# rainorangelemon/gnn-motion-planning

Measured on AMD Instinct MI355X. Metric: RGG graphs/sec (GNN explorer forward), 1000-node k=8, higher is better.
Workload: dtype f32; 1 GPU; BASELINE configs[1]: maze2, batch of 256 problems per GPU, 1000-node k1=8 RGGs (mean E=11265, O=116), loop=5, use_obstacles, real weights_maze checkpoint, fp32, sparse per-edge scores; graphs_per_gpu=256, graphs_total=256, parallelism=problem-sharded x1 (256 problems per GPU)

## Files before the change

gnn-motion-planning_amd/csrc/api.cpp:

```cpp
#include <hip/hip_runtime.h>
#include <cmath>
#include <cstdio>
#include <cstdlib>
#include <cstring>
#include <string>
#include <vector>

#include "../../include/gnnmp.h"
#include "kernels.hpp"
#include "layout.hpp"

using namespace gnnmp;

namespace {

thread_local std::string g_hip_error;

int hip_fail(hipError_t e) {
    g_hip_error = hipGetErrorString(e);
    return GNNMP_ERR_HIP;
}

#define HIP_TRY(expr)                              \
    do {                                           \
// ... 215 lines not shown
    struct Rec { int stage; hipEvent_t a, b; };
    std::vector<Rec> recs;
    std::vector<hipEvent_t> pool;
    hipEvent_t get() {
        if (!pool.empty()) { hipEvent_t e = pool.back(); pool.pop_back(); return e; }
        hipEvent_t e = nullptr;
        (void)hipEventCreate(&e);
        return e;
    }
};

struct gnnmp_explorer {
    gnnmp_explorer_dims dims;
    int device;
    float* w_dev;
    ExplorerOffsets off;
    EncBlob enc_e, enc_n;
    ObsBlob obs;
    StageProf* prof;
    int n_cu;
    int resident;
    int resident_both;
    int node_f64;
    float* w_raw_dev;
    std::vector<Entry> man;
    std::vector<int64_t> man_off;
    int64_t n_raw;
};

namespace {
struct StageScope {
    StageProf* p; hipStream_t st; hipEvent_t b = nullptr;
    StageScope(StageProf* p_, int stage, hipStream_t s) : p(p_ && p_->on ? p_ : nullptr), st(s) {
        if (!p) return;
        hipEvent_t a = p->get();
        b = p->get();
        (void)hipEventRecord(a, st);
        p->recs.push_back({stage, a, b});
    }
    ~StageScope() { if (p) (void)hipEventRecord(b, st); }
};
}

extern "C" int gnnmp_explorer_manifest(const gnnmp_explorer_dims* dims, int index, char* name, size_t name_cap,
                                       int64_t* numel) {
    if (!dims) return GNNMP_ERR_NULL;
// ... 235 lines not shown
    if (dims->embed_size == 32) {
        if (P == 2) pack_explorer<32, 2>(B, *dims, h, packed);
        else if (P == 1) pack_explorer<32, 1>(B, *dims, h, packed);
        else pack_explorer<32, 0>(B, *dims, h, packed);
    } else {
        if (P == 2) pack_explorer<64, 2>(B, *dims, h, packed);
        else if (P == 1) pack_explorer<64, 1>(B, *dims, h, packed);
        else pack_explorer<64, 0>(B, *dims, h, packed);
    }
    int prev_dev = -1;
    (void)hipGetDevice(&prev_dev);
    hipError_t e = hipSetDevice(device);
    if (e == hipSuccess) {
        int ncu = 0;
        e = hipDeviceGetAttribute(&ncu, hipDeviceAttributeMultiprocessorCount, device);
        h->n_cu = (ncu > 0 ? ncu : 256) & ~7;
        if (h->n_cu < 8) h->n_cu = 8;
        const char* env = std::getenv("GNNMP_RESIDENT");
        h->resident = !(env && env[0] == '0');
        const char* env2 = std::getenv("GNNMP_PRE_BOTH");
        h->resident_both = !(env2 && env2[0] == '0');
        const char* env3 = std::getenv("GNNMP_NODE_F64");
        h->node_f64 = !(env3 && env3[0] == '0');
    }
    if (e == hipSuccess) e = hipMalloc((void**)&h->w_dev, packed.size() * sizeof(float));
    if (e == hipSuccess) e = hipMemcpy(h->w_dev, packed.data(), packed.size() * sizeof(float), hipMemcpyHostToDevice);
    if (e == hipSuccess) e = hipMalloc((void**)&h->w_raw_dev, (size_t)tot * sizeof(float));
    if (e == hipSuccess) e = hipMemcpy(h->w_raw_dev, weights_host, (size_t)tot * sizeof(float), hipMemcpyHostToDevice);
    if (prev_dev >= 0 && prev_dev != device) (void)hipSetDevice(prev_dev);
    if (e != hipSuccess) {
        if (h->w_dev) (void)hipFree(h->w_dev);
        if (h->w_raw_dev) (void)hipFree(h->w_raw_dev);
        delete h->prof;
        delete h;
        return hip_fail(e);
    }
    *out = h;
    return GNNMP_OK;
}

extern "C" int gnnmp_explorer_destroy(gnnmp_explorer* h) {
    if (!h) return GNNMP_ERR_NULL;
    if (h->w_dev) (void)hipFree(h->w_dev);
    if (h->w_raw_dev) (void)hipFree(h->w_raw_dev);
    if (h->prof) {
        for (auto& r : h->prof->recs) { (void)hipEventDestroy(r.a); (void)hipEventDestroy(r.b); }
// ... 253 lines not shown
    const int* obs_ptr = implicit ? at<int>(ws, c.in_ptrs) + 4 : b->obs_ptr;
    {
    StageScope sc(prof, GNNMP_STAGE_PREP, st);
    q = prep_params(c, b, C, ws, implicit, use_obstacles ? 32 * c.ot_max : 0x7fffffff,
                    status_out ? reinterpret_cast<int*>(status_out) : at<int>(ws, c.gstat));
    HIP_TRY(launch_prep(q, c.Npad, c.Epad, at<int>(ws, c.prep_hist), st));
    if (dense) HIP_TRY(launch_zero_dense(dense, q.dense_ptr + c.G, st));
    if (pre_only) HIP_TRY(t_sort_csr(c.Npad, q.csr, q.row_beg, q.deg, st));
    }

    const bool use_obs = use_obstacles != 0;
    bool use_m0 = false;
    if (use_obs) {
        ObsParams op;
        op.obstacles = b->obstacles; op.obs_ptr = obs_ptr; op.S = h->dims.obs_size;
        op.w[0] = W + h->off.obs_n; op.w[1] = W + h->off.obs_e;
        op.blob = h->obs;
        op.kv[0] = at<float>(ws, c.kv_n); op.kv[1] = at<float>(ws, c.kv_e);
        op.kv_stride = c.kv_stride; op.ot_max = c.ot_max;
        NodeF64Params nq;
        nq.v = b->v; nq.C = C; nq.node_ptr = node_ptr; nq.node_ptr_pad = q.node_ptr_pad; nq.ntile_graph = q.ntile_graph;
        nq.w = W + h->off.f64; nq.blob = F64Blob::make(D, C);
        nq.m0 = at<float>(ws, c.M0);
        nq.groups = c.Npad / 64 > 2 * h->n_cu ? 4 : 1;
        {
            static const char* ord = std::getenv("GNNMP_F64_FIRST");
            nq.f64_first = ord ? (ord[0] != '0') : (nq.groups > 1 && D == 32);
        }
        nq.n_wg = (P != GNNMP_BF16 && h->node_f64) ? c.Npad / (64 * nq.groups) : 0;
        use_m0 = nq.n_wg > 0;
        StageScope sc(prof, GNNMP_STAGE_OBS, st);
        HIP_TRY(launch_obs(D, P, op, nq, c.G, st));
    }

    PreParams pp[2];
    PrePlan plan[2];
    size_t res_lds[2] = {0, 0};
    const size_t res_bytes = ((size_t)3 * (att_staged(D, P) + 6 * vec_floats(D)) + (size_t)3 * c.kv_stride) * sizeof(float) + 64 + 128;
    const bool resident_ok = ((D == 32 && P == 0) || P == 1) && use_obs && res_bytes <= 163840 && h->resident;
    for (int edge = 0; edge < 2; ++edge) {
        PreParams& p = pp[edge];
        p.v = b->v; p.goal = b->goal; p.C = C;
        p.node_ptr = node_ptr; p.node_ptr_pad = q.node_ptr_pad;
        p.tile_graph = edge ? q.etile_graph : q.ntile_graph;
        p.csr = q.csr;
        p.rec32 = at<int>(ws, c.rec32);
        p.obs_ptr = obs_ptr; p.goal_node = q.goal_node;
        p.enc = W + (edge ? h->off.enc_e : h->off.enc_n);
        p.encb = edge ? h->enc_e : h->enc_n;
        p.att = W + (edge ? h->off.att_e : h->off.att_n);
        p.out = W + (edge ? h->off.out_e : h->off.out_n);
        p.out_size = edge ? out_e_size(D, P) : out_n_size(D, P);
// ... 76 lines not shown
    }
    return GNNMP_OK;
}
}

extern "C" int gnnmp_explorer_debug_tap(const gnnmp_explorer* h, const gnnmp_batch* b, int which, float* dst, void* ws,
                                        size_t ws_bytes, void* hip_stream) {
    if (!h || !b || !dst || !ws) return GNNMP_ERR_NULL;
    Carve c;
    if (!carve(h, b, c)) return GNNMP_ERR_ARG;
    if (ws_bytes < c.total) return GNNMP_ERR_WORKSPACE;
    hipStream_t st = static_cast<hipStream_t>(hip_stream);
    const int D = h->dims.embed_size;
    size_t src;
    switch (which) {
        case 0: src = c.XI; break;
        case 1: src = c.H; break;
        case 2:
            if (h->dims.mlp_dtype == GNNMP_BF16) return GNNMP_ERR_DIMS;
            src = c.X; break;
        case 3:
            HIP_TRY(launch_goal_tap(c.G, at<int>(ws, c.goal_node), at<int>(ws, c.node_ptr_pad), dst, st));
            return GNNMP_OK;
        default: return GNNMP_ERR_ARG;
    }
    HIP_TRY(launch_unpad_rows(c.G, b->total_nodes, D, b->node_ptr ? b->node_ptr : at<int>(ws, c.in_ptrs), at<int>(ws, c.node_ptr_pad),
                              at<float>(ws, src), dst, st));
    return GNNMP_OK;
}

namespace {

std::vector<Entry> smoother_manifest(const gnnmp_smoother_dims& d) {
    const int C = d.config_size, D = d.embed_size;
    std::vector<Entry> m;
    auto lin = [&](const std::string& n, int out, int in) {
        m.push_back({n + ".weight", out, in});
        m.push_back({n + ".bias", out, 0});
    };
    lin("node_code.0", D, C + 3);
    m.push_back({"node_code.1.weight", D, 0});
    m.push_back({"node_code.1.bias", D, 0});
    m.push_back({"node_code.1.running_mean", D, 0});
    m.push_back({"node_code.1.running_var", D, 0});
    lin("node_code.3", D, D);
    lin("process.lin_0.0", D, 3 * D);
// ... 1610 lines not shown
TrainGeom to_train_geom(const gnnmp_train_geom* g) {
    TrainGeom q;
    q.G = g->n_graphs; q.C = g->config_size; q.Npad = g->n_pad; q.Epad = g->e_pad;
    q.v = g->v; q.goal = g->goal; q.node_ptr = g->node_ptr; q.node_ptr_pad = g->node_ptr_pad; q.ntile_graph = g->ntile_graph;
    q.goal_node = g->goal_node; q.row_beg = g->row_beg; q.deg = g->deg; q.csr = reinterpret_cast<const int4*>(g->csr);
    q.out_beg = g->out_beg; q.out_cnt = g->out_cnt; q.out_cur = g->out_cur; q.out_slot = g->out_slot;
    return q;
}

struct GeomCarve { Carve c; size_t obeg, ocnt, ocur, oslot, total; };
bool geom_carve(const gnnmp_batch* b, int C, GeomCarve& g) {
    (void)C;
    if (!carve(32, GNNMP_F32, b, g.c)) return false;
    size_t o = g.c.total;
    auto take = [&](size_t bytes) { const size_t r = o; o += (bytes + 255) & ~(size_t)255; return r; };
    g.obeg = take(sizeof(int) * (size_t)g.c.Npad); g.ocnt = take(sizeof(int) * (size_t)g.c.Npad);
    g.ocur = take(sizeof(int) * (size_t)g.c.Npad); g.oslot = take(sizeof(int) * (size_t)g.c.Epad);
    g.total = o;
    return true;
}

}

extern "C" int gnnmp_train_geom_workspace_bytes(const gnnmp_batch* shape, int32_t config_size, size_t* bytes) {
    if (!shape || !bytes) return GNNMP_ERR_NULL;
    if (config_size < 1) return GNNMP_ERR_ARG;
    GeomCarve g;
    if (!geom_carve(shape, config_size, g)) return GNNMP_ERR_ARG;
    *bytes = g.total;
    return GNNMP_OK;
}

extern "C" int gnnmp_train_geom_build(const gnnmp_batch* b, int32_t config_size, void* ws, size_t ws_bytes,
                                      gnnmp_train_geom* out, void* hip_stream) {
    if (!b || !ws || !out) return GNNMP_ERR_NULL;
    if (config_size < 1) return GNNMP_ERR_ARG;
    GeomCarve g;
    if (!geom_carve(b, config_size, g)) return GNNMP_ERR_ARG;
    if (!b->v || !b->goal || !b->node_ptr || !b->edge_ptr || (b->total_edges > 0 && !b->edge_index)) return GNNMP_ERR_NULL;
    if (ws_bytes < g.total || (reinterpret_cast<uintptr_t>(ws) & 255)) return GNNMP_ERR_WORKSPACE;
    hipStream_t st = static_cast<hipStream_t>(hip_stream);
    const Carve& c = g.c;
    const PrepParams q = prep_params(c, b, config_size, ws, false, 0x7fffffff, at<int>(ws, c.gstat));
    HIP_TRY(launch_prep(q, c.Npad, c.Epad, at<int>(ws, c.prep_hist), st));
    HIP_TRY(t_sort_csr(c.Npad, q.csr, q.row_beg, q.deg, st));
    out->n_graphs = c.G; out->config_size = config_size; out->n_pad = c.Npad; out->e_pad = c.Epad;
// ... 137 lines not shown
```

gnn-motion-planning_amd/csrc/explorer_kernels.hip:

```cpp
#include <hip/hip_runtime.h>
#include <cstdio>
#include <cstdlib>
#include <map>
#include <mutex>
#include <utility>
#include <math.h>
#include "chain.hpp"
#include "layout.hpp"
#include "kernels.hpp"

namespace gnnmp {

#define kETile (P == 1 ? 512 : 1024)

__device__ __forceinline__ int round_up(int x, int m) { return (x + m - 1) / m * m; }

__device__ __forceinline__ int find_graph(const int* __restrict__ ptr, int G, int x) {
    int lo = 0, hi = G;
    while (hi - lo > 1) {
        const int mid = (lo + hi) >> 1;
        if (ptr[mid] <= x) lo = mid; else hi = mid;
    }
    return lo;
}
// ... 15 lines not shown
    __syncthreads();
    if (lane == 63) wsum[wave] = x;
    __syncthreads();
    int before = 0, all = 0;
#pragma unroll
    for (int w = 0; w < 16; ++w) {
        const int t = wsum[w];
        before += w < wave ? t : 0;
        all += t;
    }
    total = all;
    return x + before;
}

__device__ __forceinline__ int prep_np(const PrepParams& q, int i) { return q.single_out ? (i > 0 ? q.single_n : 0) : q.node_ptr[i]; }
__device__ __forceinline__ int prep_ep(const PrepParams& q, int i) { return q.single_out ? (i > 0 ? q.single_e : 0) : q.edge_ptr[i]; }

__device__ __forceinline__ int prep_id(int x, int Ng, int& bad) {
    const bool b = (unsigned)x >= (unsigned)Ng;
    bad |= b ? 1 : 0;
    return b ? 0 : x;
}

__device__ __forceinline__ void prep_graph_body(const PrepParams& q, int g, int part, int parts, int n0, int Np, int e0, int e1,
                                                int* prep_lds) {
    __shared__ int carry;
    __shared__ int below_w[16];
    const int tid = threadIdx.x;
    const int c0 = prep_ep(q, g), Eg = prep_ep(q, g + 1) - c0;
    const int span = ((Np + parts - 1) / parts + 31) & ~31;
    const int lo = min(part * span, Np), hi = min(lo + span, Np), Nown = hi - lo;
    const bool in_lds = Nown <= kPrepCap;
    int* cnt = in_lds ? prep_lds : q.deg + n0 + lo;
    int* rb = in_lds ? prep_lds + kPrepCap : q.row_beg + n0 + lo;
    int* scan = prep_lds + 2 * kPrepCap;
    const long long* srcs = q.edge_index + c0;
    const long long* dsts = q.edge_index + (size_t)q.E + c0;
    for (int i = tid; i < Nown; i += 1024) cnt[i] = 0;
    __syncthreads();
    int below = 0;
    constexpr int U = 16;
    const bool in_regs = Eg <= U * 1024;
    const int Ng = prep_np(q, g + 1) - prep_np(q, g);
    int bad_id = 0;
    int sv_r[U], tv_r[U], rk_r[U];
    if (in_regs) {
#pragma unroll
        for (int u = 0; u < U; ++u) {
            const int cc = tid + u * 1024;
            const bool ok = cc < Eg;
            tv_r[u] = ok ? prep_id((int)dsts[cc], Ng, bad_id) : -1;
            sv_r[u] = ok ? prep_id((int)srcs[cc], Ng, bad_id) : 0;
        }
#pragma unroll
        for (int u = 0; u < U; ++u) {
            const int t = tv_r[u];
            below += (t >= 0 && t < lo) ? 1 : 0;
            const bool mine = t >= lo && t < hi;
// ... 3 lines not shown
    } else {
        for (int c = tid; c < Eg; c += U * 1024) {
            int d[U];
#pragma unroll
            for (int u = 0; u < U; ++u) d[u] = (c + u * 1024 < Eg) ? prep_id((int)dsts[c + u * 1024], Ng, bad_id) : 0x7fffffff;
#pragma unroll
            for (int u = 0; u < U; ++u) {
                if (d[u] < lo) ++below;
                else if (d[u] < hi) q.cursor[c0 + c + u * 1024] = atomicAdd(&cnt[d[u] - lo], 1);
            }
        }
    }
#pragma unroll
    for (int off = 32; off > 0; off >>= 1) below += __shfl_down(below, off);
    if ((tid & 63) == 0) below_w[tid >> 6] = below;
    __syncthreads();
    if (tid == 0) {
        int sum = e0;
#pragma unroll
        for (int w = 0; w < 16; ++w) sum += below_w[w];
        carry = sum;
    }
    __syncthreads();
    int carry_run = carry;
    for (int base = 0; base < Nown; base += 1024) {
        const int i = base + tid;
        const int d = (i < Nown) ? cnt[i] : 0;
        int chunk_total;
        const int incl = block_scan_1024(d, scan, chunk_total);
        if (i < Nown) {
            const int r = carry_run + incl - d;
            rb[i] = r;
            if (in_lds) { q.row_beg[n0 + lo + i] = r; q.deg[n0 + lo + i] = d; }
        }
        carry_run += chunk_total;
    }
    __syncthreads();
    if (in_regs) {
#pragma unroll
        for (int u = 0; u < U; ++u)
            if (tv_r[u] >= 0)
                q.csr[rb[tv_r[u] - lo] + rk_r[u]] = make_int4(n0 + sv_r[u], n0 + tv_r[u], c0 + tid + u * 1024, 0);
    } else {
        for (int c = tid; c < Eg; c += U * 1024) {
            int sv[U], tv[U], rk[U];
#pragma unroll
            for (int u = 0; u < U; ++u) {
                const int cc = c + u * 1024;
                tv[u] = cc < Eg ? prep_id((int)dsts[cc], Ng, bad_id) : -1;
            }
#pragma unroll
            for (int u = 0; u < U; ++u) {
                const int cc = c + u * 1024;
                const bool mine = tv[u] >= lo && tv[u] < hi;
                sv[u] = mine ? prep_id((int)srcs[cc], Ng, bad_id) : 0;
                rk[u] = mine ? q.cursor[c0 + cc] : 0;
                if (!mine) tv[u] = -1;
            }
#pragma unroll
            for (int u = 0; u < U; ++u)
                if (tv[u] >= 0)
                    q.csr[rb[tv[u] - lo] + rk[u]] = make_int4(n0 + sv[u], n0 + tv[u], c0 + c + u * 1024, 0);
        }
    }
    if (part == 0)
// ... 95 lines not shown
        an += round_up(ng, kPad);
        ae += round_up(prep_ep(q, t + 1) - prep_ep(q, t), kPad);
        ad += (long long)ng * ng;
    }
#pragma unroll
    for (int off = 32; off > 0; off >>= 1) { an += __shfl_down(an, off); ae += __shfl_down(ae, off); ad += __shfl_down(ad, off); }
    if ((tid & 63) == 0) { red[0][tid >> 6] = an; red[1][tid >> 6] = ae; red[2][tid >> 6] = ad; }
    __syncthreads();
    an = 0; ae = 0; ad = 0;
#pragma unroll
    for (int w = 0; w < 16; ++w) { an += red[0][w]; ae += red[1][w]; ad += red[2][w]; }
    const int ng_own = prep_np(q, g + 1) - prep_np(q, g);
    n0 = (int)an; e0 = (int)ae;
    n1 = n0 + round_up(ng_own, kPad); e1 = e0 + round_up(prep_ep(q, g + 1) - prep_ep(q, g), kPad);
    if (tid == 0 && part == 0) {
        if (g == 0) { q.node_ptr_pad[0] = 0; q.edge_ptr_pad[0] = 0; q.dense_ptr[0] = 0; }
        q.node_ptr_pad[g + 1] = n1; q.edge_ptr_pad[g + 1] = e1; q.dense_ptr[g + 1] = ad + (long long)ng_own * ng_own;
        const int og = q.obs_ptr ? q.obs_ptr[g + 1] - q.obs_ptr[g] : q.single_o;
        q.gstat[kGstatStride * g] = og > q.obs_cap ? 1 : 0;
        for (int pp = parts; pp < kGstatStride - 1; ++pp) q.gstat[kGstatStride * g + 1 + pp] = 0;
    }
}

__device__ __forceinline__ void prep_trailing(const PrepParams& q, int n_end, int e_end, int Npad, int Epad) {
    const int tid = threadIdx.x;
    for (int i = n_end + tid; i < Npad; i += 1024) { q.deg[i] = 0; q.row_beg[i] = e_end; }
    for (int t = n_end / 32 + tid; t < Npad / 32; t += 1024) q.ntile_graph[t] = -1;
    for (int t = e_end / 32 + tid; t < Epad / 32; t += 1024) { q.etile_graph[t] = -1; q.tile_meta[t] = -1; }
    for (int sl = e_end + tid; sl < Epad; sl += 1024) q.csr[sl] = make_int4(-1, -1, -1, -1);
}

__global__ __launch_bounds__(1024) void prep_small_kernel(PrepParams q, int Npad, int Epad, int parts) {
    extern __shared__ int prep_lds[];
    const int g = blockIdx.x / parts, part = blockIdx.x - g * parts;
    int n0, n1, e0, e1;
    prep_prefix<false>(q, g, part, parts, n0, n1, e0, e1);
    prep_graph_body(q, g, part, parts, n0, n1 - n0, e0, e1, prep_lds);
    if (part == 0) goal_body(q.C, q.v, q.goal, prep_np(q, g), prep_np(q, g + 1) - prep_np(q, g), g, n0, q.goal_node);
    if (g == q.G - 1 && part == parts - 1) prep_trailing(q, n1, e1, Npad, Epad);
}

__global__ __launch_bounds__(1024) void prep_hist_kernel(PrepParams q, int Npad, int Epad, int parts, int* __restrict__ H) {
    extern __shared__ int prep_lds[];
    const int idx = blockIdx.x >> 3, g = (idx / parts) * 8 + (blockIdx.x & 7), part = idx % parts, tid = threadIdx.x;
    if (g >= q.G) return;
    int n0, n1, e0, e1;
    prep_prefix<true>(q, g, part, parts, n0, n1, e0, e1);
    const int Np = n1 - n0;
    const int c0 = q.edge_ptr[g], Eg = q.edge_ptr[g + 1] - c0;
    const int cs = (int)((long long)Eg * part / parts), ce = (int)((long long)Eg * (part + 1) / parts);
    int* hslice = H + (size_t)n0 * parts + (size_t)part * Np;
    const bool in_lds = Np <= kPrepCap;
    int* cnt = in_lds ? prep_lds : hslice;
    const long long* dsts = q.edge_index + (size_t)q.E + c0;
    for (int i = tid; i < Np; i += 1024) cnt[i] = 0;
    __syncthreads();
    constexpr int U = 16;
    const int Ng = q.node_ptr[g + 1] - q.node_ptr[g];
    int bad_id = 0;
    for (int c = cs + tid; c < ce; c += U * 1024) {
        int d[U];
#pragma unroll
// ... 296 lines not shown
                y[ob] = __builtin_amdgcn_mfma_f64_16x16x4f64((double)A[((ob * NB + ib) * 4 + st) * 64 + lane], x[ib][st], y[ob], 0, 0, 0);
            if constexpr (NB > 2) __builtin_amdgcn_sched_barrier(0);
        }
}

template <int NB>
__device__ __forceinline__ void vec64(const float* b, f64x4 (&y)[NB], int g) {
#pragma unroll
    for (int ob = 0; ob < NB; ++ob)
#pragma unroll
        for (int r = 0; r < 4; ++r) y[ob][r] = (double)b[16 * ob + 4 * r + g];
}

template <int D, int P>
__device__ __forceinline__ void node_f64_body(const ObsParams& p, const NodeF64Params& q, const int vblock) {
    constexpr int NB = D / 16, NT = D / 32, OC = f64_obs_chunk(D);
    extern __shared__ __attribute__((aligned(16))) float lds[];
    const F64Blob L = q.blob;
    float* wl = lds;
    float* kd = lds + ((L.size + 3) & ~3);
    float* vd = kd + OC * D;
    const int wave = threadIdx.x >> 6, lane = threadIdx.x & 63, j16 = lane & 15, g = lane >> 4;
    const int row00 = vblock * 64 * q.groups;
    const int gr = q.ntile_graph[row00 >> 5];
    if (gr < 0) return;
    stage(wl, q.w, L.size);
    const int o0 = p.obs_ptr[gr], O = min(p.obs_ptr[gr + 1] - o0, p.ot_max * 32);
    const int OT = (O + 31) / 32;
    const int C = q.C;
    const int nbase_pad = q.node_ptr_pad[gr], nbase = q.node_ptr[gr], ng = q.node_ptr[gr + 1] - nbase;
    const bool single_chunk = O <= OC;
    const double isd = 1.0 / sqrt((double)D);
    for (int grp = 0; grp < q.groups; ++grp) {
    const int row0 = row00 + grp * 64;
    if (row0 - nbase_pad >= ng) {
        for (int i = threadIdx.x; i < (q.groups - grp) * 64 * D; i += 256) q.m0[(size_t)row0 * D + i] = 0.f;
        break;
    }
    const int row = row0 + wave * 16 + j16, local = row - nbase_pad;
    const float* vr = q.v + (size_t)(nbase + (local < ng ? local : 0)) * C;

    f64x4 x[NB], acc[NB];
    float xf[NB][4];
    float mxs = 0.f, l0s = 0.f;
    double den = 0.0;
    for (int oc0 = 0; oc0 == 0 || oc0 < O; oc0 += OC) {
        if (oc0 > 0 || (grp > 0 && !single_chunk)) __syncthreads();
        if (grp == 0 || !single_chunk)
        {
            const ObsBlob Lo = p.blob;
            const int h = lane >> 5, j = lane & 31, S = p.S;
            for (int ot = (oc0 >> 5) + wave; ot < min(OT, (oc0 + OC) >> 5); ot += 4) {
                const float* W = p.w[0];
                asm volatile("" : "+s"(W));
                const int o = ot * 32 + j;
                const bool valid = o < O;
                const float* orow = p.obstacles + (size_t)(o0 + (valid ? o : 0)) * S;
                f32x16 code[NT], K[NT], V[NT];
                mlp2_in<NT, P>(W + Lo.as0, Lo.ks, W + Lo.b0, W + Lo.a0, W + Lo.c0,
                               [&](int k) { const bool ok = k < S; const float xx = orow[ok ? k : 0]; return ok ? xx : 0.f; }, code, lane);
#pragma unroll
                for (int t = 0; t < NT; ++t) { K[t] = splat16(0.f); V[t] = splat16(0.f); }
                linear_acc_p<P, NT, NT>(W + Lo.blk0 + Lo.wk, code, K, lane);
                linear_acc_p<P, NT, NT>(W + Lo.blk0 + Lo.wv, code, V, lane);
                const int oo = o - oc0;
                float* kb = kd + (oo >> 4) * NB * 256 + (oo & 15) + 64 * h;
                float* vb = vd + (oo >> 4) * NB * 256 + (oo & 3) * 64 + 16 * ((oo & 15) >> 2) + 4 * h;
#pragma unroll
                for (int t = 0; t < NT; ++t)
#pragma unroll
                    for (int r = 0; r < 16; ++r) {
                        const int f0 = 32 * t + phi(r, 0);
                        kb[(f0 >> 4) * 256 + ((f0 & 15) >> 2) * 64 + 16 * (f0 & 3)] = valid ? K[t][r] : 0.f;
                        vb[(f0 >> 4) * 256 + (f0 & 15)] = valid ? V[t][r] : 0.f;
                    }
            }
        }
        if (grp == 0 || !single_chunk) __syncthreads();
        if (oc0 == 0) {
            f64x4 hdn[NB];
            vec64<NB>(wl + L.b1, hdn, g);
            for (int st = 0; st < L.ks; ++st) {
                const int k = 4 * st + g;
                const double xin = k < C ? (double)vr[k] : 0.0;
#pragma unroll
                for (int ob = 0; ob < NB; ++ob)
                    hdn[ob] = __builtin_amdgcn_mfma_f64_16x16x4f64((double)wl[L.w1 + (ob * L.ks + st) * 64 + lane], xin, hdn[ob], 0, 0, 0);
            }
#pragma unroll
            for (int ob = 0; ob < NB; ++ob)
#pragma unroll
                for (int r = 0; r < 4; ++r) hdn[ob][r] = fmax(hdn[ob][r], 0.0);
            vec64<NB>(wl + L.b2, x, g);
            lin64<NB>(wl + L.w2, hdn, x, lane);
#pragma unroll
            for (int ob = 0; ob < NB; ++ob)
#pragma unroll
                for (int r = 0; r < 4; ++r) xf[ob][r] = (float)x[ob][r];
            f32x4 tq[NB], mv[NB];
#pragma unroll
            for (int ob = 0; ob < NB; ++ob) { tq[ob] = f32x4{0.f, 0.f, 0.f, 0.f}; mv[ob] = f32x4{0.f, 0.f, 0.f, 0.f}; }
// ... 1784 lines not shown
template <class K>
static hipError_t set_lds(K kernel, size_t bytes) {
    return hipFuncSetAttribute(reinterpret_cast<const void*>(kernel), hipFuncAttributeMaxDynamicSharedMemorySize,
                               (int)bytes);
}

int prep_parts(int G, int E) {
    static const int parts_env = getenv("GNNMP_PREP_PARTS") ? atoi(getenv("GNNMP_PREP_PARTS")) : 0;
    const long long g = G > 0 ? G : 1;
    long long parts = (long long)E / (g * kPrepEdgesPerPart);
    if (parts > 256 / g) parts = 256 / g;
    if (parts > 1) {
        long long fine = (long long)E / (g * (kPrepEdgesPerPart / 2));
        if (fine > 512 / g) fine = 512 / g;
        if (fine > 8) fine = 8;
        if (fine > parts) parts = fine;
    }
    if (parts_env > 0) parts = parts_env;
    if (parts < 1) parts = 1;
    if (parts > kPrepMaxParts) parts = kPrepMaxParts;
    return (int)parts;
}

hipError_t launch_prep(const PrepParams& q, int Npad, int Epad, int* hist, hipStream_t st) {
    const size_t glds = (size_t)(2 * kPrepCap + 1024) * sizeof(int);
    const int parts = prep_parts(q.G, q.E);
    if (parts == 1) {
        const hipError_t attr = set_lds(prep_small_kernel, glds);
        if (attr != hipSuccess) return attr;
        static const int slices_env = getenv("GNNMP_PREP_SLICES") ? atoi(getenv("GNNMP_PREP_SLICES")) : 0;
        int slices = q.G > 0 ? 512 / q.G : 1;
        const int by_nodes = q.G > 0 ? (Npad / q.G) / 128 : 1;
        if (slices > by_nodes) slices = by_nodes;
        if (slices > 8) slices = 8;
        if (slices_env > 0) slices = slices_env;
        if (slices < 1) slices = 1;
        if (slices > kGstatStride - 1) slices = kGstatStride - 1;
        hipLaunchKernelGGL(prep_small_kernel, dim3(q.G * slices), dim3(1024), glds, st, q, Npad, Epad, slices);
        LAUNCH_CHECK();
        return hipSuccess;
    }
    hipError_t attr = set_lds(prep_hist_kernel, glds);
    if (attr != hipSuccess) return attr;
    attr = set_lds(prep_scatter_kernel, glds);
    if (attr != hipSuccess) return attr;
    const unsigned grid = (unsigned)(((q.G + 7) / 8) * 8 * parts);
    hipLaunchKernelGGL(prep_hist_kernel, dim3(grid), dim3(1024), glds, st, q, Npad, Epad, parts, hist);
    LAUNCH_CHECK();
    hipLaunchKernelGGL(prep_scatter_kernel, dim3(grid), dim3(1024), glds, st, q, parts, hist, hist + (size_t)parts * Npad);
    LAUNCH_CHECK();
    return hipSuccess;
}


template <int D, int P>
static hipError_t launch_obs_t(const ObsParams& p, const NodeF64Params& q, int G, hipStream_t st) {
    const int f64_blocks = P == 1 ? 0 : q.n_wg;
    size_t lds = f64_blocks ? (size_t)(((q.blob.size + 3) & ~3) + 2 * f64_obs_chunk(D) * D) * sizeof(float) : 0;
    const size_t obs_lds = (D == 32 && P != 2) ? (size_t)((p.blob.size + 3) & ~3) * sizeof(float) : 0;
    if (obs_lds > lds) lds = obs_lds;
    if (lds) {
        const hipError_t e = set_lds(obs_kernel<D, P>, lds);
        if (e != hipSuccess) return e;
    }
    hipLaunchKernelGGL((obs_kernel<D, P>), dim3(f64_blocks + 2 * G), dim3(256), lds, st, p, q, f64_blocks);
    LAUNCH_CHECK();
    return hipSuccess;
}
#define GNNMP_DISPATCH_DP(D_, P_, CALL)                                                     \
    do {                                                                                     \
        if ((D_) == 32 && (P_) == 0) { constexpr int DD = 32, PP = 0; return CALL; }         \
        if ((D_) == 32 && (P_) == 1) { constexpr int DD = 32, PP = 1; return CALL; }         \
        if ((D_) == 32 && (P_) == 2) { constexpr int DD = 32, PP = 2; return CALL; }         \
        if ((D_) == 64 && (P_) == 0) { constexpr int DD = 64, PP = 0; return CALL; }         \
        if ((D_) == 64 && (P_) == 1) { constexpr int DD = 64, PP = 1; return CALL; }         \
        if ((D_) == 64 && (P_) == 2) { constexpr int DD = 64, PP = 2; return CALL; }         \
        return hipErrorInvalidValue;                                                         \
    } while (0)

hipError_t launch_obs(int D, int P, const ObsParams& p, const NodeF64Params& q, int G, hipStream_t st) {
    GNNMP_DISPATCH_DP(D, P, (launch_obs_t<DD, PP>(p, q, G, st)));
}

// ... 43 lines not shown
    return hipErrorInvalidValue;
}
hipError_t launch_pre_resident(int D, int P, bool edge, const PreParams& p, size_t lds_bytes, int n_cu, hipStream_t st) {
    if (D == 32 && P == 0) return edge ? launch_pre_resident_t<32, 0, true, 12>(p, lds_bytes, n_cu, st) : launch_pre_resident_t<32, 0, false, 12>(p, lds_bytes, n_cu, st);
    if (D == 32 && P == 1) return edge ? launch_pre_resident_t<32, 1, true, 12>(p, lds_bytes, n_cu, st) : launch_pre_resident_t<32, 1, false, 12>(p, lds_bytes, n_cu, st);
    if (D == 64 && P == 1) return edge ? launch_pre_resident_t<64, 1, true, 12>(p, lds_bytes, n_cu, st) : launch_pre_resident_t<64, 1, false, 8>(p, lds_bytes, n_cu, st);
    return hipErrorInvalidValue;
}

struct Residency { int per_cu, cus; };
static Residency resident_workgroups(const void* kernel, size_t lds_bytes) {
    static std::mutex mu;
    static std::map<std::pair<const void*, size_t>, Residency> cache;
    std::lock_guard<std::mutex> lock(mu);
    auto it = cache.find({kernel, lds_bytes});
    if (it != cache.end()) return it->second;
    Residency r{0, 256};
    int dev = 0;
    hipDeviceProp_t prop;
    if (hipGetDevice(&dev) == hipSuccess && hipGetDeviceProperties(&prop, dev) == hipSuccess) r.cus = prop.multiProcessorCount;
    if (hipOccupancyMaxActiveBlocksPerMultiprocessor(&r.per_cu, kernel, 256, lds_bytes) != hipSuccess || r.per_cu < 1) r.per_cu = 4;
    if (getenv("GNNMP_DEBUG_GRID")) fprintf(stderr, "[gnnmp] resident workgroups per CU: %d (lds %zu)\n", r.per_cu, lds_bytes);
    return cache[{kernel, lds_bytes}] = r;
}

template <class K>
static int grid_for(K kernel, size_t lds_bytes, int n_tiles, int max_per_cu) {
    int groups = ((n_tiles + 3) / 4 + 7) & ~7;
    if (groups < 8) groups = 8;
    const Residency r = resident_workgroups(reinterpret_cast<const void*>(kernel), lds_bytes);
    int per_cu = r.per_cu < max_per_cu ? r.per_cu : max_per_cu;
    static const int forced = getenv("GNNMP_WGS_PER_CU") ? atoi(getenv("GNNMP_WGS_PER_CU")) : 0;
    if (forced > 0) per_cu = forced;
    const int cap = (r.cus * per_cu) & ~7;
    return groups < cap ? groups : (cap < 8 ? 8 : cap);
}

#ifdef GNNMP_MP_TRACE
static long long* g_mp_trace = nullptr;
static size_t g_mp_trace_n = 0;
extern "C" long long gnnmp_debug_mp_trace(long long* dst, long long cap) {
    if (!g_mp_trace) return 0;
    const size_t n = g_mp_trace_n < (size_t)cap ? g_mp_trace_n : (size_t)cap;
    (void)hipDeviceSynchronize();
    (void)hipMemcpy(dst, g_mp_trace, n * sizeof(long long), hipMemcpyDeviceToHost);
    return (long long)n;
// ... 147 lines not shown
```

gnn-motion-planning_amd/csrc/kernels.hpp:

```cpp
#pragma once
#include <hip/hip_runtime.h>
#include "layout.hpp"

namespace gnnmp {

struct PrepParams {
    int G, E, C;
    const long long* edge_index;
    const int *node_ptr, *edge_ptr;
    const float *v, *goal;
    int *node_ptr_pad, *edge_ptr_pad;
    long long* dense_ptr;
    int *deg, *cursor, *row_beg;
    int *ntile_graph, *etile_graph;
    int4* csr;
    int* goal_node;
    int* tile_meta;
    int2* blk_span;
    int* single_out;
    int single_n, single_e, single_o;
    int n_etiles;
    const int* obs_ptr;
    int obs_cap;
    int* gstat;
};
constexpr int kGstatStride = 17;

struct ObsParams {
    const float* obstacles;
    const int* obs_ptr;
    int S;
    const float* w[2];
    ObsBlob blob;
    float* kv[2];
    int kv_stride;
    int ot_max;
};

struct NodeF64Params {
    const float* v;
    int C;
    const int *node_ptr, *node_ptr_pad, *ntile_graph;
    const float* w;
    F64Blob blob;
    float* m0;
    int n_wg;
    int f64_first;
    int groups;
};

struct PreParams {
    const float *v, *goal;
    int C;
    const int *node_ptr, *node_ptr_pad;
    const int* tile_graph;
    const int4* csr;
    int* rec32;
    const int* obs_ptr;
    const int* goal_node;
    const float* enc;
    EncBlob encb;
    const float* att;
    const float* out;
    int out_size;
    const float* kv;
    int kv_stride, ot_max, ot_chunk;
    int wregion;
    int n_wg;
// ... 288 lines not shown
    int B, A;
    int P, Nn, Ec;
};
hipError_t t_sm_nodes_in_seg(const SmSeg& g, int C, float scale, const float* cur, const float* free_pts, const float* coll, float* out,
                             hipStream_t st);
hipError_t t_bn_seg_fwd(const SmSeg& g, int D, const float* x, const float* gamma, const float* beta, float* y, float* stats,
                        float* out_stats, size_t out_stride, bool relu, hipStream_t st);
hipError_t t_bn_seg_bwd(const SmSeg& g, int D, const float* x, const float* dy, const float* gamma, const float* stats, float* dx,
                        float* part, hipStream_t st);
hipError_t t_bn_seg_dgb(int L, int B, int D, const float* part, float* dgamma, float* dbeta, hipStream_t st);
hipError_t t_sm_msg_in_seg(const SmSeg& g, const int* n_edges, int D, const int* e_src, const int* e_dst, const float* X, float* out,
                           hipStream_t st);
hipError_t t_sm_msg_in_bwd_seg(const SmSeg& g, const int* n_edges, int D, const int* e_src, const int* e_dst, const float* dZ, float* dX,
                               hipStream_t st);
hipError_t t_sm_scatter_add_seg(const SmSeg& g, const int* n_edges, int D, const int* e_dst, const float* M, float* S, hipStream_t st);
hipError_t t_sm_scatter_add_bwd_seg(const SmSeg& g, const int* n_edges, int D, const int* e_dst, const float* dS, float* dM, hipStream_t st);
hipError_t t_sm_add_path_seg(const SmSeg& g, int D, const float* X, const float* Y, float* out, hipStream_t st);
hipError_t t_sm_add_path_bwd_seg(const SmSeg& g, int D, const float* dH, float* dX, hipStream_t st);
hipError_t t_sm_path_update_seg(const SmSeg& g, int C, const float* prev, const float* proposal, float* next, hipStream_t st);
hipError_t t_sm_path_update_bwd_seg(const SmSeg& g, int C, const float* d_next, float* d_proposal, float* d_prev, hipStream_t st);
hipError_t t_sm_coords_bwd_seg(const SmSeg& g, int C, const float* dXin, float* d_prev, hipStream_t st);

int prep_parts(int G, int E);
hipError_t launch_prep(const PrepParams& q, int Npad, int Epad, int* hist, hipStream_t st);
hipError_t launch_obs(int D, int P, const ObsParams& p, const NodeF64Params& q, int G, hipStream_t st);
hipError_t launch_pre(int D, int P, bool edge, int waves, const PreParams& p, int n_tiles32, size_t lds_bytes, hipStream_t st);
hipError_t launch_pre_resident_both(int D, int P, const PreParams& pn, const PreParams& pe, size_t lds_bytes, int node_blocks,
                                    int edge_blocks, hipStream_t st);
hipError_t launch_pre_resident(int D, int P, bool edge, const PreParams& p, size_t lds_bytes, int n_cu, hipStream_t st);
hipError_t launch_mp_fused(int D, int P, const MpFusedParams& p, hipStream_t st);
hipError_t launch_policy(int D, int P, const PolicyParams& p, hipStream_t st);
hipError_t launch_unpad_rows(int G, int total_nodes, int D, const int* node_ptr, const int* node_ptr_pad,
                             const float* src, float* dst, hipStream_t st);
hipError_t launch_zero_dense(float* dense, const long long* n_ptr, hipStream_t st);
hipError_t launch_goal_tap(int G, const int* goal_node, const int* node_ptr_pad, float* dst, hipStream_t st);

}
```

include/gnnmp.h:

```cpp
#ifndef GNNMP_H
#define GNNMP_H

#include <stddef.h>
#include <stdint.h>

#ifdef __cplusplus
extern "C" {
#endif

typedef enum {
    GNNMP_OK = 0,
    GNNMP_ERR_NULL = -1,
    GNNMP_ERR_DIMS = -2,
    GNNMP_ERR_WEIGHTS = -3,
    GNNMP_ERR_WORKSPACE = -4,
    GNNMP_ERR_HIP = -5,
    GNNMP_ERR_ARG = -6,
    GNNMP_ERR_CAPS = -7,
    GNNMP_ERR_INDEX = -8
} gnnmp_status;

const char* gnnmp_status_string(int status);
const char* gnnmp_last_hip_error(void);
int gnnmp_abi_version(void);
// ... 297 lines not shown
enum {
    GNNMP_TOP_LINEAR = 0, GNNMP_TOP_LINEAR_DX, GNNMP_TOP_LINEAR_DW, GNNMP_TOP_RELU_BWD, GNNMP_TOP_FILL,
    GNNMP_TOP_NODE_IN, GNNMP_TOP_EDGE_IN, GNNMP_TOP_H0, GNNMP_TOP_H0_BWD, GNNMP_TOP_CONCAT, GNNMP_TOP_SPLIT,
    GNNMP_TOP_MSG_IN, GNNMP_TOP_MSG_IN_BWD, GNNMP_TOP_POL_IN, GNNMP_TOP_POL_IN_BWD, GNNMP_TOP_SEGMENT_MAX,
    GNNMP_TOP_SEGMENT_MAX_BWD, GNNMP_TOP_SCORES_OUT, GNNMP_TOP_SCORES_IN, GNNMP_TOP_SM_NODES_IN, GNNMP_TOP_BN_FWD,
    GNNMP_TOP_BN_BWD, GNNMP_TOP_SM_MSG_IN, GNNMP_TOP_SM_MSG_IN_BWD, GNNMP_TOP_SM_SCATTER_ADD,
    GNNMP_TOP_SM_SCATTER_ADD_BWD, GNNMP_TOP_ADD_ROWS, GNNMP_TOP_SM_PATH_UPDATE, GNNMP_TOP_SM_PATH_UPDATE_BWD,
    GNNMP_TOP_SM_COORDS_BWD, GNNMP_TOP_SCALE,
    GNNMP_TOP_SM_NODES_IN_SEG, GNNMP_TOP_BN_SEG_FWD, GNNMP_TOP_BN_SEG_BWD, GNNMP_TOP_BN_SEG_DGB, GNNMP_TOP_SM_MSG_IN_SEG,
    GNNMP_TOP_SM_MSG_IN_BWD_SEG, GNNMP_TOP_SM_SCATTER_ADD_SEG, GNNMP_TOP_SM_SCATTER_ADD_BWD_SEG, GNNMP_TOP_SM_ADD_PATH_SEG,
    GNNMP_TOP_SM_ADD_PATH_BWD_SEG, GNNMP_TOP_SM_PATH_UPDATE_SEG, GNNMP_TOP_SM_PATH_UPDATE_BWD_SEG, GNNMP_TOP_SM_COORDS_BWD_SEG,
    GNNMP_TOP_FINAL_CAT, GNNMP_TOP_SEED_DH, GNNMP_TOP_LINEAR_DW_ORDER, GNNMP_TOP_COUNT
};

typedef struct {
    int32_t n_graphs, config_size, n_pad, e_pad;
    const float *v, *goal;
    const int32_t *node_ptr, *node_ptr_pad, *ntile_graph, *goal_node, *row_beg, *deg;
    const int32_t* csr;
    int32_t *out_beg, *out_cnt, *out_cur, *out_slot;
} gnnmp_train_geom;

int gnnmp_train_geom_workspace_bytes(const gnnmp_batch* shape, int32_t config_size, size_t* bytes);
int gnnmp_train_geom_build(const gnnmp_batch* batch, int32_t config_size, void* workspace, size_t workspace_bytes,
                           gnnmp_train_geom* geom_out, void* hip_stream);
int gnnmp_train_op(int op, const int64_t* dims, int n_dims, void* const* bufs, int n_bufs,
                   const gnnmp_train_geom* geom_or_null, float scalar, void* hip_stream);
int64_t gnnmp_train_dw_scratch_floats(int64_t R, int64_t K, int64_t O);
int gnnmp_train_op_path(int op, const int64_t* dims, int n_dims);

int64_t gnnmp_pack_a_tiles(const float* w, int out_f, int ld, int col0, int n_in, float* dst);
int64_t gnnmp_pack_a_small(const float* w, int out_f, int ld, int col0, int n_in, float* dst);
int64_t gnnmp_pack_vec(const float* b, int n, float* dst);
int64_t gnnmp_pack_f64_ops(const float* w, int out_f, int ld, int col0, int n_in, int row_perm, float* dst);

#ifdef __cplusplus
}
#endif
#endif
```

Baseline: 83950 graphs/s.

## Stage CSR records in LDS, spread trailing fill, and tune f64 obs grouping

The prep kernel now buffers each slice's CSR records as packed int2 entries in LDS, then writes them out to global memory in coalesced order instead of scattering them. It also uses a smaller counter capacity template when slices are small, and halves the default slice count in that mode. Every workgroup now computes the trailing padding bounds and shares the fill work, where before the last block did it alone. The obs/f64 kernel can now span multiple graphs per workgroup, with a group count chosen from an occupancy-based wave cost model. The trade-offs are more LDS per prep block, an extra cross-graph reduction in every block, and more complex group bookkeeping.

```diff
diff --git a/gnn-motion-planning_amd/csrc/api.cpp b/gnn-motion-planning_amd/csrc/api.cpp
--- a/gnn-motion-planning_amd/csrc/api.cpp
+++ b/gnn-motion-planning_amd/csrc/api.cpp
@@ -261,6 +261,7 @@
     int resident;
     int resident_both;
     int node_f64;
+    int f64_groups;
     float* w_raw_dev;
     std::vector<Entry> man;
     std::vector<int64_t> man_off;
@@ -542,6 +543,9 @@
         h->resident_both = !(env2 && env2[0] == '0');
         const char* env3 = std::getenv("GNNMP_NODE_F64");
         h->node_f64 = !(env3 && env3[0] == '0');
+        const char* env4 = std::getenv("GNNMP_F64_GROUPS");
+        const int fg = env4 ? std::atoi(env4) : 0;
+        h->f64_groups = (fg == 1 || (fg >= 4 && fg <= 16 && fg % 4 == 0)) ? fg : 0;
     }
     if (e == hipSuccess) e = hipMalloc((void**)&h->w_dev, packed.size() * sizeof(float));
     if (e == hipSuccess) e = hipMemcpy(h->w_dev, packed.data(), packed.size() * sizeof(float), hipMemcpyHostToDevice);
@@ -841,12 +845,25 @@
         nq.v = b->v; nq.C = C; nq.node_ptr = node_ptr; nq.node_ptr_pad = q.node_ptr_pad; nq.ntile_graph = q.ntile_graph;
         nq.w = W + h->off.f64; nq.blob = F64Blob::make(D, C);
         nq.m0 = at<float>(ws, c.M0);
+        nq.n_rows = c.Npad;
+        const bool f64_role = P != GNNMP_BF16 && h->node_f64;
         nq.groups = c.Npad / 64 > 2 * h->n_cu ? 4 : 1;
+        if (nq.groups == 4 && f64_role) {
+            const int slots = obs_f64_slots(D, P, op, nq);
+            const long long per_graph = ((long long)b->total_nodes / c.G + kPad - 1) / kPad;
+            const long long blocks = per_graph * c.G;
+            long long best = 0;
+            for (int m = 1; m <= 4 && slots > 0; m *= 2) {
+                const long long wgs = (blocks + m - 1) / m, cost = (wgs + slots - 1) / slots * m;
+                if (m == 1 || cost <= best) { best = cost; nq.groups = 4 * m; }
+            }
+        }
+        if (h->f64_groups) nq.groups = h->f64_groups;
         {
             static const char* ord = std::getenv("GNNMP_F64_FIRST");
             nq.f64_first = ord ? (ord[0] != '0') : (nq.groups > 1 && D == 32);
         }
-        nq.n_wg = (P != GNNMP_BF16 && h->node_f64) ? c.Npad / (64 * nq.groups) : 0;
+        nq.n_wg = f64_role ? (c.Npad + 64 * nq.groups - 1) / (64 * nq.groups) : 0;
         use_m0 = nq.n_wg > 0;
         StageScope sc(prof, GNNMP_STAGE_OBS, st);
         HIP_TRY(launch_obs(D, P, op, nq, c.G, st));
@@ -969,6 +986,9 @@
         case 3:
             HIP_TRY(launch_goal_tap(c.G, at<int>(ws, c.goal_node), at<int>(ws, c.node_ptr_pad), dst, st));
             return GNNMP_OK;
+        case 4:
+            if (h->dims.mlp_dtype == GNNMP_BF16 || !h->node_f64) return GNNMP_ERR_DIMS;
+            src = c.M0; break;
         default: return GNNMP_ERR_ARG;
     }
     HIP_TRY(launch_unpad_rows(c.G, b->total_nodes, D, b->node_ptr ? b->node_ptr : at<int>(ws, c.in_ptrs), at<int>(ws, c.node_ptr_pad),
@@ -2625,6 +2645,8 @@
 
 }
 
+extern "C" int gnnmp_prep_lds_row_capacity(int32_t nodes_per_slice) { return prep_lds_row_capacity(nodes_per_slice); }
+
 extern "C" int gnnmp_train_geom_workspace_bytes(const gnnmp_batch* shape, int32_t config_size, size_t* bytes) {
     if (!shape || !bytes) return GNNMP_ERR_NULL;
     if (config_size < 1) return GNNMP_ERR_ARG;
diff --git a/gnn-motion-planning_amd/csrc/explorer_kernels.hip b/gnn-motion-planning_amd/csrc/explorer_kernels.hip
--- a/gnn-motion-planning_amd/csrc/explorer_kernels.hip
+++ b/gnn-motion-planning_amd/csrc/explorer_kernels.hip
@@ -61,18 +61,23 @@
     return b ? 0 : x;
 }
 
+__host__ __device__ constexpr int prep_row_capacity(int lds_ints, int cap) {
+    return lds_ints > 2 * cap + 1024 ? (lds_ints - 2 * cap - 1024) / 2 : 0;
+}
+
+template <int CAP>
 __device__ __forceinline__ void prep_graph_body(const PrepParams& q, int g, int part, int parts, int n0, int Np, int e0, int e1,
-                                                int* prep_lds) {
+                                                int* prep_lds, int rec_cap) {
     __shared__ int carry;
     __shared__ int below_w[16];
     const int tid = threadIdx.x;
     const int c0 = prep_ep(q, g), Eg = prep_ep(q, g + 1) - c0;
     const int span = ((Np + parts - 1) / parts + 31) & ~31;
     const int lo = min(part * span, Np), hi = min(lo + span, Np), Nown = hi - lo;
-    const bool in_lds = Nown <= kPrepCap;
+    const bool in_lds = Nown <= CAP;
     int* cnt = in_lds ? prep_lds : q.deg + n0 + lo;
-    int* rb = in_lds ? prep_lds + kPrepCap : q.row_beg + n0 + lo;
-    int* scan = prep_lds + 2 * kPrepCap;
+    int* rb = in_lds ? prep_lds + CAP : q.row_beg + n0 + lo;
+    int* scan = prep_lds + 2 * CAP;
     const long long* srcs = q.edge_index + c0;
     const long long* dsts = q.edge_index + (size_t)q.E + c0;
     for (int i = tid; i < Nown; i += 1024) cnt[i] = 0;
@@ -122,7 +127,8 @@
         carry = sum;
     }
     __syncthreads();
-    int carry_run = carry;
+    int carry_run = __builtin_amdgcn_readfirstlane(carry);
+    const int slot0 = carry_run;
     for (int base = 0; base < Nown; base += 1024) {
         const int i = base + tid;
         const int d = (i < Nown) ? cnt[i] : 0;
@@ -133,14 +139,27 @@
             rb[i] = r;
             if (in_lds) { q.row_beg[n0 + lo + i] = r; q.deg[n0 + lo + i] = d; }
         }
-        carry_run += chunk_total;
+        carry_run += __builtin_amdgcn_readfirstlane(chunk_total);
     }
     __syncthreads();
+    const int own = carry_run - slot0;
+    const bool rows = q.lds_rows && in_lds && Ng <= 65536 && own <= rec_cap;
     if (in_regs) {
+        int2* rec = reinterpret_cast<int2*>(scan + 1024);
 #pragma unroll
         for (int u = 0; u < U; ++u)
-            if (tv_r[u] >= 0)
-                q.csr[rb[tv_r[u] - lo] + rk_r[u]] = make_int4(n0 + sv_r[u], n0 + tv_r[u], c0 + tid + u * 1024, 0);
+            if (tv_r[u] >= 0) {
+                const int slot = rb[tv_r[u] - lo] + rk_r[u];
+                if (rows) rec[slot - slot0] = make_int2((int)((unsigned)sv_r[u] | ((unsigned)tv_r[u] << 16)), tid + u * 1024);
+                else q.csr[slot] = make_int4(n0 + sv_r[u], n0 + tv_r[u], c0 + tid + u * 1024, 0);
+            }
+        if (rows) {
+            __syncthreads();
+            for (int i = tid; i < own; i += 1024) {
+                const int2 r = rec[i];
+                q.csr[slot0 + i] = make_int4(n0 + (r.x & 0xffff), n0 + (int)((unsigned)r.x >> 16), c0 + r.y, 0);
+            }
+        }
     } else {
         for (int c = tid; c < Eg; c += U * 1024) {
             int sv[U], tv[U], rk[U];
@@ -282,22 +301,44 @@
     }
 }
 
-__device__ __forceinline__ void prep_trailing(const PrepParams& q, int n_end, int e_end, int Npad, int Epad) {
+__device__ __forceinline__ void prep_end(const PrepParams& q, int g, int n1, int e1, int& n_end, int& e_end) {
+    __shared__ int tot[2][16];
     const int tid = threadIdx.x;
-    for (int i = n_end + tid; i < Npad; i += 1024) { q.deg[i] = 0; q.row_beg[i] = e_end; }
-    for (int t = n_end / 32 + tid; t < Npad / 32; t += 1024) q.ntile_graph[t] = -1;
-    for (int t = e_end / 32 + tid; t < Epad / 32; t += 1024) { q.etile_graph[t] = -1; q.tile_meta[t] = -1; }
-    for (int sl = e_end + tid; sl < Epad; sl += 1024) q.csr[sl] = make_int4(-1, -1, -1, -1);
-}
-
-__global__ __launch_bounds__(1024) void prep_small_kernel(PrepParams q, int Npad, int Epad, int parts) {
-    extern __shared__ int prep_lds[];
+    int tn = 0, te = 0;
+    for (int t = g + 1 + tid; t < q.G; t += 1024) {
+        tn += round_up(prep_np(q, t + 1) - prep_np(q, t), kPad);
+        te += round_up(prep_ep(q, t + 1) - prep_ep(q, t), kPad);
+    }
+#pragma unroll
+    for (int off = 32; off > 0; off >>= 1) { tn += __shfl_down(tn, off); te += __shfl_down(te, off); }
+    if ((tid & 63) == 0) { tot[0][tid >> 6] = tn; tot[1][tid >> 6] = te; }
+    __syncthreads();
+    tn = n1; te = e1;
+#pragma unroll
+    for (int w = 0; w < 16; ++w) { tn += tot[0][w]; te += tot[1][w]; }
+    n_end = tn; e_end = te;
+}
+
+__device__ __forceinline__ void prep_trailing(const PrepParams& q, int n_end, int e_end, int Npad, int Epad, int wg = 0, int nwg = 1) {
+    const int tid = wg * 1024 + threadIdx.x, nt = nwg * 1024;
+    for (int i = n_end + tid; i < Npad; i += nt) { q.deg[i] = 0; q.row_beg[i] = e_end; }
+    for (int t = n_end / 32 + tid; t < Npad / 32; t += nt) q.ntile_graph[t] = -1;
+    for (int t = e_end / 32 + tid; t < Epad / 32; t += nt) { q.etile_graph[t] = -1; q.tile_meta[t] = -1; }
+    for (int sl = e_end + tid; sl < Epad; sl += nt) q.csr[sl] = make_int4(-1, -1, -1, -1);
+}
+
+template <int CAP>
+__global__ __launch_bounds__(1024) void prep_small_kernel(PrepParams q, int Npad, int Epad, int parts, int rec_cap) {
+    extern __shared__ __attribute__((aligned(16))) int prep_lds[];
     const int g = blockIdx.x / parts, part = blockIdx.x - g * parts;
-    int n0, n1, e0, e1;
+    int n0, n1, e0, e1, n_end, e_end;
     prep_prefix<false>(q, g, part, parts, n0, n1, e0, e1);
-    prep_graph_body(q, g, part, parts, n0, n1 - n0, e0, e1, prep_lds);
+    n0 = __builtin_amdgcn_readfirstlane(n0); n1 = __builtin_amdgcn_readfirstlane(n1);
+    e0 = __builtin_amdgcn_readfirstlane(e0); e1 = __builtin_amdgcn_readfirstlane(e1);
+    prep_graph_body<CAP>(q, g, part, parts, n0, n1 - n0, e0, e1, prep_lds, rec_cap);
     if (part == 0) goal_body(q.C, q.v, q.goal, prep_np(q, g), prep_np(q, g + 1) - prep_np(q, g), g, n0, q.goal_node);
-    if (g == q.G - 1 && part == parts - 1) prep_trailing(q, n1, e1, Npad, Epad);
+    prep_end(q, g, n1, e1, n_end, e_end);
+    prep_trailing(q, n_end, e_end, Npad, Epad, (int)blockIdx.x, (int)gridDim.x);
 }
 
 __global__ __launch_bounds__(1024) void prep_hist_kernel(PrepParams q, int Npad, int Epad, int parts, int* __restrict__ H) {
@@ -640,20 +681,28 @@
     float* vd = kd + OC * D;
     const int wave = threadIdx.x >> 6, lane = threadIdx.x & 63, j16 = lane & 15, g = lane >> 4;
     const int row00 = vblock * 64 * q.groups;
-    const int gr = q.ntile_graph[row00 >> 5];
-    if (gr < 0) return;
+    if (row00 >= q.n_rows || q.ntile_graph[row00 >> 5] < 0) return;
     stage(wl, q.w, L.size);
-    const int o0 = p.obs_ptr[gr], O = min(p.obs_ptr[gr + 1] - o0, p.ot_max * 32);
-    const int OT = (O + 31) / 32;
     const int C = q.C;
-    const int nbase_pad = q.node_ptr_pad[gr], nbase = q.node_ptr[gr], ng = q.node_ptr[gr + 1] - nbase;
-    const bool single_chunk = O <= OC;
     const double isd = 1.0 / sqrt((double)D);
+    int gr = -1, o0 = 0, O = 0, OT = 0, nbase_pad = 0, nbase = 0, ng = 0;
+    bool single_chunk = true, used = false;
     for (int grp = 0; grp < q.groups; ++grp) {
     const int row0 = row00 + grp * 64;
+    const int gnew = row0 < q.n_rows ? q.ntile_graph[row0 >> 5] : -1;
+    if (gnew < 0) break;
+    const bool fresh = gnew != gr;
+    if (fresh) {
+        gr = gnew;
+        o0 = p.obs_ptr[gr]; O = min(p.obs_ptr[gr + 1] - o0, p.ot_max * 32);
+        OT = (O + 31) / 32;
+        nbase_pad = q.node_ptr_pad[gr]; nbase = q.node_ptr[gr]; ng = q.node_ptr[gr + 1] - nbase;
+        single_chunk = O <= OC;
+    }
     if (row0 - nbase_pad >= ng) {
-        for (int i = threadIdx.x; i < (q.groups - grp) * 64 * D; i += 256) q.m0[(size_t)row0 * D + i] = 0.f;
-        break;
+        for (int i = threadIdx.x; i < 64 * D; i += 256) q.m0[(size_t)row0 * D + i] = 0.f;
+        if (fresh) gr = -1;
+        continue;
     }
     const int row = row0 + wave * 16 + j16, local = row - nbase_pad;
     const float* vr = q.v + (size_t)(nbase + (local < ng ? local : 0)) * C;
@@ -663,8 +712,9 @@
     float mxs = 0.f, l0s = 0.f;
     double den = 0.0;
     for (int oc0 = 0; oc0 == 0 || oc0 < O; oc0 += OC) {
-        if (oc0 > 0 || (grp > 0 && !single_chunk)) __syncthreads();
-        if (grp == 0 || !single_chunk)
+        const bool build = fresh || !single_chunk;
+        if (build && used) __syncthreads();
+        if (build)
         {
             const ObsBlob Lo = p.blob;
             const int h = lane >> 5, j = lane & 31, S = p.S;
@@ -694,7 +744,8 @@
                     }
             }
         }
-        if (grp == 0 || !single_chunk) __syncthreads();
+        if (build) __syncthreads();
+        used = true;
         if (oc0 == 0) {
             f64x4 hdn[NB];
             vec64<NB>(wl + L.b1, hdn, g);
@@ -2525,21 +2576,42 @@
     return (int)parts;
 }
 
-hipError_t launch_prep(const PrepParams& q, int Npad, int Epad, int* hist, hipStream_t st) {
+constexpr int kPrepSmallLdsInts = (160 * 1024 - 1024) / (int)sizeof(int);
+static_assert(kPrepSmallLdsInts >= 2 * kPrepCap + 1024, "counters of kPrepCap own nodes + scan");
+constexpr int kPrepCapSmall = 2048;
+static int prep_counter_cap(int nodes_per_slice) { return nodes_per_slice <= kPrepCapSmall * 3 / 4 ? kPrepCapSmall : kPrepCap; }
+
+int prep_lds_row_capacity(int nodes_per_slice) { return prep_row_capacity(kPrepSmallLdsInts, prep_counter_cap(nodes_per_slice)); }
+
+hipError_t launch_prep(const PrepParams& q_in, int Npad, int Epad, int* hist, hipStream_t st) {
     const size_t glds = (size_t)(2 * kPrepCap + 1024) * sizeof(int);
+    PrepParams q = q_in;
+    {
+        const char* env = getenv("GNNMP_PREP_LDS_ROWS");
+        q.lds_rows = !(env && env[0] == '0');
+    }
     const int parts = prep_parts(q.G, q.E);
     if (parts == 1) {
-        const hipError_t attr = set_lds(prep_small_kernel, glds);
-        if (attr != hipSuccess) return attr;
+        const size_t slds = (size_t)kPrepSmallLdsInts * sizeof(int);
         static const int slices_env = getenv("GNNMP_PREP_SLICES") ? atoi(getenv("GNNMP_PREP_SLICES")) : 0;
-        int slices = q.G > 0 ? 512 / q.G : 1;
+        int slices = q.G > 0 ? (q.lds_rows ? 256 : 512) / q.G : 1;
         const int by_nodes = q.G > 0 ? (Npad / q.G) / 128 : 1;
         if (slices > by_nodes) slices = by_nodes;
         if (slices > 8) slices = 8;
         if (slices_env > 0) slices = slices_env;
         if (slices < 1) slices = 1;
         if (slices > kGstatStride - 1) slices = kGstatStride - 1;
-        hipLaunchKernelGGL(prep_small_kernel, dim3(q.G * slices), dim3(1024), glds, st, q, Npad, Epad, slices);
+        const int cap = prep_counter_cap(q.G > 0 ? Npad / q.G / slices : Npad);
+        const int rec_cap = prep_row_capacity(kPrepSmallLdsInts, cap);
+        if (cap == kPrepCapSmall) {
+            const hipError_t attr = set_lds(prep_small_kernel<kPrepCapSmall>, slds);
+            if (attr != hipSuccess) return attr;
+            hipLaunchKernelGGL(prep_small_kernel<kPrepCapSmall>, dim3(q.G * slices), dim3(1024), slds, st, q, Npad, Epad, slices, rec_cap);
+        } else {
+            const hipError_t attr = set_lds(prep_small_kernel<kPrepCap>, slds);
+            if (attr != hipSuccess) return attr;
+            hipLaunchKernelGGL(prep_small_kernel<kPrepCap>, dim3(q.G * slices), dim3(1024), slds, st, q, Npad, Epad, slices, rec_cap);
+        }
         LAUNCH_CHECK();
         return hipSuccess;
     }
@@ -2557,11 +2629,16 @@
 
 
 template <int D, int P>
+static size_t obs_lds_bytes(const ObsParams& p, const NodeF64Params& q, bool f64_role) {
+    size_t lds = f64_role ? (size_t)(((q.blob.size + 3) & ~3) + 2 * f64_obs_chunk(D) * D) * sizeof(float) : 0;
+    const size_t obs_lds = (D == 32 && P != 2) ? (size_t)((p.blob.size + 3) & ~3) * sizeof(float) : 0;
+    return obs_lds > lds ? obs_lds : lds;
+}
+
+template <int D, int P>
 static hipError_t launch_obs_t(const ObsParams& p, const NodeF64Params& q, int G, hipStream_t st) {
     const int f64_blocks = P == 1 ? 0 : q.n_wg;
-    size_t lds = f64_blocks ? (size_t)(((q.blob.size + 3) & ~3) + 2 * f64_obs_chunk(D) * D) * sizeof(float) : 0;
-    const size_t obs_lds = (D == 32 && P != 2) ? (size_t)((p.blob.size + 3) & ~3) * sizeof(float) : 0;
-    if (obs_lds > lds) lds = obs_lds;
+    const size_t lds = obs_lds_bytes<D, P>(p, q, f64_blocks > 0);
     if (lds) {
         const hipError_t e = set_lds(obs_kernel<D, P>, lds);
         if (e != hipSuccess) return e;
@@ -2651,6 +2728,19 @@
     if (hipOccupancyMaxActiveBlocksPerMultiprocessor(&r.per_cu, kernel, 256, lds_bytes) != hipSuccess || r.per_cu < 1) r.per_cu = 4;
     if (getenv("GNNMP_DEBUG_GRID")) fprintf(stderr, "[gnnmp] resident workgroups per CU: %d (lds %zu)\n", r.per_cu, lds_bytes);
     return cache[{kernel, lds_bytes}] = r;
+}
+
+template <int D, int P>
+static int obs_f64_slots_t(const ObsParams& p, const NodeF64Params& q) {
+    const Residency r = resident_workgroups(reinterpret_cast<const void*>(obs_kernel<D, P>), obs_lds_bytes<D, P>(p, q, true));
+    return r.per_cu * r.cus;
+}
+int obs_f64_slots(int D, int P, const ObsParams& p, const NodeF64Params& q) {
+    if (D == 32 && P == 0) return obs_f64_slots_t<32, 0>(p, q);
+    if (D == 32 && P == 2) return obs_f64_slots_t<32, 2>(p, q);
+    if (D == 64 && P == 0) return obs_f64_slots_t<64, 0>(p, q);
+    if (D == 64 && P == 2) return obs_f64_slots_t<64, 2>(p, q);
+    return 0;
 }
 
 template <class K>
diff --git a/gnn-motion-planning_amd/csrc/kernels.hpp b/gnn-motion-planning_amd/csrc/kernels.hpp
--- a/gnn-motion-planning_amd/csrc/kernels.hpp
+++ b/gnn-motion-planning_amd/csrc/kernels.hpp
@@ -23,6 +23,7 @@
     const int* obs_ptr;
     int obs_cap;
     int* gstat;
+    int lds_rows;
 };
 constexpr int kGstatStride = 17;
 
@@ -44,6 +45,7 @@
     const float* w;
     F64Blob blob;
     float* m0;
+    int n_rows;
     int n_wg;
     int f64_first;
     int groups;
@@ -378,8 +380,10 @@
 hipError_t t_sm_coords_bwd_seg(const SmSeg& g, int C, const float* dXin, float* d_prev, hipStream_t st);
 
 int prep_parts(int G, int E);
+int prep_lds_row_capacity(int nodes_per_slice);
 hipError_t launch_prep(const PrepParams& q, int Npad, int Epad, int* hist, hipStream_t st);
 hipError_t launch_obs(int D, int P, const ObsParams& p, const NodeF64Params& q, int G, hipStream_t st);
+int obs_f64_slots(int D, int P, const ObsParams& p, const NodeF64Params& q);
 hipError_t launch_pre(int D, int P, bool edge, int waves, const PreParams& p, int n_tiles32, size_t lds_bytes, hipStream_t st);
 hipError_t launch_pre_resident_both(int D, int P, const PreParams& pn, const PreParams& pe, size_t lds_bytes, int node_blocks,
                                     int edge_blocks, hipStream_t st);
diff --git a/include/gnnmp.h b/include/gnnmp.h
--- a/include/gnnmp.h
+++ b/include/gnnmp.h
@@ -343,6 +343,7 @@
 } gnnmp_train_geom;
 
 int gnnmp_train_geom_workspace_bytes(const gnnmp_batch* shape, int32_t config_size, size_t* bytes);
+int gnnmp_prep_lds_row_capacity(int32_t nodes_per_slice);
 int gnnmp_train_geom_build(const gnnmp_batch* batch, int32_t config_size, void* workspace, size_t workspace_bytes,
                            gnnmp_train_geom* geom_out, void* hip_stream);
 int gnnmp_train_op(int op, const int64_t* dims, int n_dims, void* const* bufs, int n_bufs,
```

After: 85110 graphs/s, median of 6. 1.4% higher.
